# amolrpatil21/PorQua

Hardware: AMD Instinct MI355X
Metric: QPs solved/sec (rebalance dates) at N=1000 assets, 1-8 GPU; x vs host CPU (higher is better)
Workload: dtype f64; 1 GPU; config3: long-only min-variance (P=2*Pearson cov, budget + box [0,1]), daily rebalance; n_assets=1000, window=252, dates_per_gpu=4749, global_batch=4749, parallelism=dates-sharded x1

## Files before the change

### include/porqua_hip.h

```cpp
#ifndef PORQUA_HIP_H
#define PORQUA_HIP_H

#include <stdint.h>

#ifdef __cplusplus
extern "C" {
#endif

#define PQ_VERSION 100

#define PQ_UNSOLVED 0
#define PQ_SOLVED 1
#define PQ_SOLVED_INACCURATE 2
#define PQ_MAX_ITER 3
#define PQ_NEED_REFACTOR 4
#define PQ_PRIMAL_INFEASIBLE (-3)
#define PQ_DUAL_INFEASIBLE (-4)
#define PQ_NON_CONVEX (-5)

#define PQ_OUT_OBJ 0
#define PQ_OUT_PRIM 1
#define PQ_OUT_DUAL 2
#define PQ_OUT_GAP 3
#define PQ_OUT_RHO 4
// ... 137 lines not shown
int pq_admm_lr_grouped(const pq_lowrank* lr, const pq_problem* pb, pq_state* st, const double* Minv,
                       int32_t k_ld, int64_t M_stride, const int32_t* gdates, int32_t ngroups,
                       const int32_t* urows, const int32_t* ucnt, const int32_t* uoff, int32_t umax,
                       const pq_settings* s, int32_t iters_this_call, const double* pc, int64_t ldpc,
                       int32_t r0, const double* cc, const int32_t* cg_nzr, const double* cg_nzv,
                       int32_t nzmax, void* stream);

int pq_admm_lr_sweep(const pq_lowrank* lr, const pq_problem* pb, pq_state* st, const double* Minv,
                     int32_t k_ld, int64_t M_stride, const int32_t* gdates, int32_t ngroups,
                     const pq_settings* s, int32_t iters_this_call, const double* pc, int64_t ldpc,
                     int32_t r0, const double* cc, int32_t q_shared, double* scratch, int64_t scratch_doubles,
                     void* stream);
int64_t pq_sweep_scratch_doubles(int32_t n, int32_t batch, int32_t ngroups);

typedef struct pq_gcap {
  const int32_t* gdates; int32_t ngroups;
  const int32_t* urows; const int32_t* ucnt; const int32_t* uoff; int32_t umax;
  const int32_t* gidx;
  double* grho;
  double* M; double* Minv; int32_t k_ld; int64_t M_stride;
  double* aq; int64_t aq_stride;
  double* hinv; int32_t ldh;
  int32_t gmax;
} pq_gcap;
int pq_gcap_assemble(const pq_lowrank* lr, const pq_problem* pb, const pq_gcap* gc, const pq_settings* s,
                     const double* band, int64_t ldo, int32_t r0, const double* pc, int64_t ldpc,
                     const double* cc, void* stream);
int pq_gcap_prepare(const pq_lowrank* lr, const pq_problem* pb, pq_state* st, const pq_gcap* gc,
                    const pq_settings* s, const int32_t* idx, int32_t nidx, const double* band, int64_t ldo,
                    int32_t r0, const double* pc, int64_t ldpc, void* stream);
int pq_admm_lr_gcap(const pq_lowrank* lr, const pq_problem* pb, pq_state* st, const pq_gcap* gc,
                    const pq_settings* s, int32_t iters_this_call, const double* pc, int64_t ldpc, int32_t r0,
                    const double* cc, const int32_t* cg_nzr, const double* cg_nzv, int32_t nzmax, void* stream);

int pq_eigcap_form(const pq_lowrank* lr, const pq_problem* pb, const pq_state* st, const pq_settings* s,
                   const int32_t* pdate, const double* V, const double* evals, const double* What,
                   const double* cc, int32_t k_ld, const int32_t* idx, int32_t nidx, double* Minv,
                   int64_t M_stride, double* scratch, void* stream);

int pq_polish_batched(const pq_problem* pb, pq_state* st, const int32_t* idx, int32_t nidx,
                      const pq_settings* s, void* stream);

int pq_polish_lr_batched(const pq_lowrank* lr, const pq_problem* pb, pq_state* st,
                         const int32_t* idx, int32_t nidx, const pq_settings* s, void* stream);

int pq_polish_w_batched(const pq_lowrank* lr, const pq_problem* pb, pq_state* st, const int32_t* idx,
                        int32_t nidx, const pq_settings* s, int32_t ldk, int32_t final_try,
                        const double* band, int64_t ldo, int32_t r0, void* stream);

#define PQ_PG_RECORD 384
#define PQ_PG_PASS_SCRATCH 123537
#define PQ_PG_PENDING 0
#define PQ_PG_DONE 1
#define PQ_PG_FALLBACK 2
#define PQ_PG_SKIP 3
#define PQ_PG_WMB 8
#define PQ_PG_WSCR(k_ld) (2 * PQ_PG_WMB * (int64_t)(k_ld))
typedef struct pq_pg_wide {
  const pq_gcap* gc;
  const double* pc; int64_t ldpc; int32_t r0; const double* cc;
  const int32_t* nzr; const double* nzv; int32_t nzmax;
  double* wscr; int64_t wscr_stride;
  int32_t refine_steps;
} pq_pg_wide;
int pq_polish_grouped_init(const pq_lowrank* lr, const pq_problem* pb, pq_state* st, double* rec,
                           const pq_settings* s, void* stream);
// ... 97 lines not shown
```

### porqua_amd/_lib.py

```python
from __future__ import annotations

import ctypes
import os

_HERE = os.path.dirname(os.path.abspath(__file__))
LIB_PATH = os.environ.get("PQ_LIB_PATH") or os.path.join(_HERE, "libporqua_hip.so")

c_int32 = ctypes.c_int32
c_int64 = ctypes.c_int64
c_dp = ctypes.c_void_p

PQ_UNSOLVED = 0
PQ_SOLVED = 1
PQ_SOLVED_INACCURATE = 2
PQ_MAX_ITER = 3
PQ_NEED_REFACTOR = 4
PQ_PRIMAL_INFEASIBLE = -3
PQ_DUAL_INFEASIBLE = -4
PQ_NON_CONVEX = -5

PQ_PCT_OK, PQ_PCT_EMPTY_BUCKET, PQ_PCT_NAN_SCORE = range(3)
PQ_PCT_MAX_N = 16384
PQ_PCT_MAX_BUCKETS = 256

# ... 161 lines not shown
    "pq_admm_lr_grouped": ([ctypes.POINTER(PQLowRank), ctypes.POINTER(PQProblem), ctypes.POINTER(PQState),
                            c_dp, c_int32, c_int64, c_dp, c_int32, c_dp, c_dp, c_dp, c_int32,
                            ctypes.POINTER(PQSettings), c_int32, c_dp, c_int64, c_int32, c_dp, c_dp, c_dp,
                            c_int32, c_dp], c_int32),
    "pq_admm_lr_sweep": ([ctypes.POINTER(PQLowRank), ctypes.POINTER(PQProblem), ctypes.POINTER(PQState),
                          c_dp, c_int32, c_int64, c_dp, c_int32, ctypes.POINTER(PQSettings), c_int32, c_dp,
                          c_int64, c_int32, c_dp, c_int32, c_dp, c_int64, c_dp], c_int32),
    "pq_sweep_scratch_doubles": ([c_int32, c_int32, c_int32], c_int64),
    "pq_polish_lr_batched": ([ctypes.POINTER(PQLowRank), ctypes.POINTER(PQProblem), ctypes.POINTER(PQState),
                              c_dp, c_int32, ctypes.POINTER(PQSettings), c_dp], c_int32),
    "pq_lr_capacitance": ([ctypes.POINTER(PQLowRank), ctypes.POINTER(PQProblem), ctypes.POINTER(PQState),
                           c_dp, c_int32, ctypes.POINTER(PQSettings), c_dp, c_int32, c_int64, c_dp], c_int32),
    "pq_lr_band_gram": ([c_dp, c_int64, c_int32, c_int32, c_int32, c_int32, c_dp, c_int64, c_dp, c_int32, c_int32,
                         c_dp, c_int64, c_dp], c_int32),
    "pq_lr_capacitance_band": ([ctypes.POINTER(PQLowRank), ctypes.POINTER(PQProblem), ctypes.POINTER(PQState),
                                c_dp, c_int32, ctypes.POINTER(PQSettings), c_dp, c_int64, c_int32, c_dp, c_int64,
                                c_dp, c_dp, c_int32, c_int64, c_dp], c_int32),
    "pq_admm_lr_batched": ([ctypes.POINTER(PQLowRank), ctypes.POINTER(PQProblem), ctypes.POINTER(PQState),
                            c_dp, c_int32, c_int64, c_dp, c_int32, ctypes.POINTER(PQSettings), c_int32,
                            c_dp], c_int32),
    "pq_polish_grouped_init": ([ctypes.POINTER(PQLowRank), ctypes.POINTER(PQProblem), ctypes.POINTER(PQState),
                                c_dp, ctypes.POINTER(PQSettings), c_dp], c_int32),
    "pq_polish_grouped_round": ([ctypes.POINTER(PQLowRank), ctypes.POINTER(PQProblem), ctypes.POINTER(PQState),
                                 c_dp, c_int32, c_dp, c_int32, c_dp, c_dp, c_dp, c_int32,
                                 ctypes.POINTER(PQSettings), c_dp, ctypes.POINTER(PQPgWide), c_dp], c_int32),
    "pq_gcap_assemble": ([ctypes.POINTER(PQLowRank), ctypes.POINTER(PQProblem), ctypes.POINTER(PQGcap),
                          ctypes.POINTER(PQSettings), c_dp, c_int64, c_int32, c_dp, c_int64, c_dp, c_dp], c_int32),
    "pq_gcap_prepare": ([ctypes.POINTER(PQLowRank), ctypes.POINTER(PQProblem), ctypes.POINTER(PQState),
                         ctypes.POINTER(PQGcap), ctypes.POINTER(PQSettings), c_dp, c_int32, c_dp, c_int64, c_int32,
                         c_dp, c_int64, c_dp], c_int32),
    "pq_admm_lr_gcap": ([ctypes.POINTER(PQLowRank), ctypes.POINTER(PQProblem), ctypes.POINTER(PQState),
                         ctypes.POINTER(PQGcap), ctypes.POINTER(PQSettings), c_int32, c_dp, c_int64, c_int32, c_dp,
                         c_dp, c_dp, c_int32, c_dp], c_int32),
    "pq_eigcap_form": ([ctypes.POINTER(PQLowRank), ctypes.POINTER(PQProblem), ctypes.POINTER(PQState),
                        ctypes.POINTER(PQSettings), c_dp, c_dp, c_dp, c_dp, c_dp, c_int32, c_dp, c_int32, c_dp,
                        c_int64, c_dp, c_dp], c_int32),
    "pq_gemv_batched": ([c_dp, c_int64, c_int64, c_int32, c_int32, c_int32, c_int32, c_dp, c_int64, c_dp,
                         c_int64, c_dp], c_int32),
    "pq_workspace_bytes": ([c_int32, c_int32, c_int32, c_int32, c_int32, c_int32], c_int64),
    "pq_simulate_periods": ([c_dp, c_int64, c_int32, c_dp, c_int64, c_dp, c_dp, c_int32, c_dp, c_dp,
                             ctypes.c_double, ctypes.c_double, c_dp, c_dp, c_int64, c_dp, c_int32, c_dp], c_int32),
    "pq_lad_mv_batched": ([c_dp, c_int64, c_int64, c_int32, c_int32, c_dp, c_int64, c_int32, c_dp, c_int64,
                           c_dp, c_int64, c_dp], c_int32),
    "pq_wgram_batched": ([c_dp, c_int64, c_int64, c_int32, c_int32, c_int32, c_dp, c_int64, c_dp, c_int64,
                          c_dp, c_int64, c_dp, c_int32, c_int64, c_dp], c_int32),
    "pq_percentile_batched": ([c_dp, c_int64, c_int32, c_int32, ctypes.c_double, c_int32, c_dp, c_dp, c_dp,
                               c_dp, c_dp, c_dp, c_dp, c_dp, c_dp], c_int32),
    "pq_shrink_stats_band": ([c_dp, c_int64, c_int32, c_int32, c_int32, c_dp, c_int64, c_dp, c_int32, c_int32,
                              c_int32, c_int32, c_int32, c_dp, c_dp], c_int32),
    "pq_risk_parity_batched": ([ctypes.POINTER(PQLowRank), c_int32, c_int32, c_dp, c_dp, c_dp, c_int64,
                                ctypes.c_double, ctypes.c_double, c_int32, c_dp, c_int64, c_dp, c_dp, c_dp],
                               c_int32),
    "pq_hrp_batched": ([c_dp, c_int64, c_int32, c_int32, c_dp, c_dp, ctypes.c_double, c_dp, c_int64, c_dp, c_int64,
                        c_dp, c_dp, c_dp, c_dp], c_int32),
    "pq_hrp_linkage_batched": ([c_dp, c_int64, c_int32, c_int32, c_dp, c_dp, ctypes.c_double, c_int32, c_dp, c_int64,
                                c_dp, c_int64, c_dp, c_int64, c_dp, c_dp, c_dp, c_dp], c_int32),
    "pq_window_gram_batched": ([c_dp, c_int64, c_int32, c_dp, c_dp, c_int32, c_int32, c_dp, c_int64, c_dp, c_int32,
                                c_int64, c_dp], c_int32),
    "pq_window_project_batched": ([c_dp, c_int64, c_int32, c_dp, c_dp, c_int32, c_int32, c_dp, c_int64, c_dp,
                                   c_int32, c_int64, c_dp, c_dp, c_dp, c_int32, c_dp, c_dp, c_int64, c_dp], c_int32),
}

_lib = None


def load() -> ctypes.CDLL:
# ... 25 lines not shown
```

### porqua_amd/csrc/admm_gcap.hip

```cpp
#include "admm_dev.h"
#include "chol_dev.h"
#include "capi_util.h"

namespace pq {

constexpr int CT = 256;
constexpr int CNW = CT / 64;
constexpr int CHW = CT / 32;
constexpr int CTP1 = 5;
constexpr int CTP2 = 6;
constexpr int CG_MAX = 16;
constexpr int CU_MAX = 320;
constexpr int CMG = 4;
constexpr int CMGW = 24;
constexpr int CNZ = 4;
constexpr int CP1_ROWS = 16 * CNW * CTP1;
constexpr int CK_MAX = CP1_ROWS + 4;
constexpr int CH_MAX = 64;

#ifdef PQ_PROFILE
#define CSTAMP(k)                                                 \
  do {                                                            \
    __syncthreads();                                              \
    if (threadIdx.x == 0) {                                       \
// ... 364 lines not shown
      const int i = e >> 6, j = e & 63;
      T64[i * DP + j] = (i < mh && j < mh) ? h_entry(gg, i, j) : (i == j ? 1.0 : 0.0);
    }
    if (tile_chol_inv64(T64, X64, mh)) {
      if (t == 0) st.status[b] = PQ_NON_CONVEX;
      continue;
    }
    double* Hi = gc.hinv + (int64_t)b * gc.ldh * gc.ldh;
    const int ldh = gc.ldh;
    const int cc = l & 15, g4 = l >> 4;
    for (int tt = w; tt < 10; tt += PW_PREP) {
      int I = 0;
      while ((I + 1) * (I + 2) / 2 <= tt) ++I;
      const int J = tt - I * (I + 1) / 2;
      f64x4 acc = f64x4{0.0, 0.0, 0.0, 0.0};
#pragma unroll 4
      for (int k0 = 0; k0 < TB; k0 += 4)
        acc = __builtin_amdgcn_mfma_f64_16x16x4f64(X64[(16 * I + cc) * DP + k0 + g4], X64[(16 * J + cc) * DP + k0 + g4],
                                                  acc, 0, 0, 0);
#pragma unroll
      for (int q = 0; q < 4; ++q) {
        const int i = 16 * I + g4 + 4 * q, j = 16 * J + cc;
        const bool in = i < mh && j < mh;
        if (i < ldh && j < ldh) Hi[(int64_t)i * ldh + j] = in ? acc[q] : 0.0;
        if (I != J && i < ldh && j < ldh) Hi[(int64_t)j * ldh + i] = in ? acc[q] : 0.0;
      }
    }
  }
}

#ifndef PQ_GCAP_SKIP1
#define PQ_GCAP_SKIP1 1
#endif
template <int MGC, int NB>
__global__ __launch_bounds__(CT * NB) __attribute__((amdgpu_waves_per_eu(2, 2))) void k_admm_gcap(pq_lowrank lr, pq_problem pb, pq_state st, pq_gcap gc,
                                                  pq_settings s, int iters_call, const double* pc, int64_t ldpc,
                                                  int r0, const double* cc, const int32_t* cg_nzr,
                                                  const double* cg_nzv, int nzmax) {
  constexpr bool WIDE = MGC > CMG;
  constexpr int MGG = WIDE ? CMGW : 8;
  constexpr int CTN = CT * NB, CNWN = CTN / 64, CHWN = CTN / 32;
  constexpr int CG = CG_MAX * NB;
  constexpr int CTP1N = (CP1_ROWS / 16 + CNWN - 1) / CNWN;
  constexpr int CTP2N = ((CK_MAX + 15) / 16 + CNWN - 1) / CNWN;
  static_assert(CTP1N * CNWN * 16 >= CP1_ROWS && CTP2N * CNWN * 16 >= CK_MAX, "k_admm_gcap tiling");
  __shared__ __attribute__((aligned(16))) double WU[(CU_MAX + 4) * CG];
  double* const UT = WU;
  __shared__ double g_muv[CG], g_su[CG], g_dinv[CG], g_rn[CG], g_qmax[CG], g_coef[CG];
  __shared__ double g_y[CG * CH_MAX];
  constexpr int NPART = 5;
  __shared__ double g_part[CNWN * CG_MAX * NPART];
  __shared__ double g_gm[CG * 3];
  __shared__ double g_zg[CG * MGG], g_yg[CG * MGG], g_cgv[CG * MGG], g_cgx[CG * MGG],
      g_wg[CG * MGG], g_cw[CG * MGG], g_rgz[CG * MGG], g_cmu[CG * MGG];
  __shared__ double g_rg[MGG], g_lg[MGG], g_ug[MGG];
  double* const g_zt = g_rgz;
  __shared__ int g_act[CG], g_it[CG], g_end[CG], g_stat[CG], g_off[CG], g_T[CG];
  __shared__ int s_urow[CU_MAX];
  __shared__ double s_sr[MGG];
  __shared__ double s_rho;
  __shared__ int s_any;

  const int grp = xcd_slot(blockIdx.x, gridDim.x);
  const int d0 = gc.gdates[grp];
  const int G = gc.gdates[grp + 1] - d0;
  const int U = gc.ucnt[grp];
  const int t = threadIdx.x, w = wave_id(), l = lane_id();
  const int n = pb.n, ld = pb.ld, mg = pb.mg, k_ld = gc.k_ld;
  const int kU = U + mg;
  const bool has_box = pb.lb != nullptr;
  const bool centred = lr.mu != nullptr;
  const double sigma = s.sigma, alpha = s.alpha;
  const double* Mi = gc.Minv + (int64_t)grp * gc.M_stride;
#ifdef PQ_PROFILE
  long long pclk[5] = {0, 0, 0, 0, 0};
  long long tclk = wall_clock64();
#endif

  if (kU > CP1_ROWS || U > CU_MAX || G > CG || kU > k_ld) {
    for (int g = t; g < G; g += CTN) st.status[d0 + g] = PQ_NON_CONVEX;
    return;
  }

  for (int u = t; u < CU_MAX; u += CTN) s_urow[u] = u < U ? gc.urows[(int64_t)grp * gc.umax + u] : 0;
  for (int e = t; e < (CU_MAX + 4) * CG; e += CTN) UT[e] = 0.0;
  if (t == 0) s_rho = gc.grho[grp];
  __syncthreads();
  const double rho = s_rho;
  const GConst gk = gconst(lr, pb, s, d0, rho);
  if (t < mg) s_sr[t] = sqrt(row_rho(pb.lg[t], pb.ug[t], rho, s));
  if (t < CG) {
    const int g = t;
    int act = 0;
    if (g < G) {
      const int b = d0 + g;
      const int stt = st.status[b];
      act = (stt == PQ_UNSOLVED || stt == PQ_NEED_REFACTOR);
      g_it[g] = st.iters[b];
      g_end[g] = min(s.max_iter, st.iters[b] + iters_call);
      g_stat[g] = stt;
      g_T[g] = lr.tlen[b];
      g_off[g] = gc.uoff[b];
      g_dinv[g] = 1.0 / gk.d;
    }
    g_act[g] = act;
  }
  for (int e = t; e < CG * MGG; e += CTN) {
    const int g = e / MGG, r = e % MGG;
    double zg = 0, yg = 0;
    if (g < G && r < mg) {
      const int b = d0 + g;
      zg = st.z[(int64_t)b * st.m_ld + r];
      yg = st.y[(int64_t)b * st.m_ld + r];
    }
    g_zg[e] = zg;
    g_yg[e] = yg;
  }
  if (t < MGG) {
    const bool ok = t < mg;
    g_lg[t] = ok ? pb.lg[t] : 0.0;
    g_ug[t] = ok ? pb.ug[t] : 0.0;
    g_rg[t] = ok ? row_rho(pb.lg[t], pb.ug[t], rho, s) : 0.0;
// ... 63 lines not shown
      }
    }
    muv = lanes_sum<32>(muv);
    qmax = lanes_max<32>(qmax);
#pragma unroll
    for (int r = 0; r < CMG; ++r) cvp[r] = lanes_sum<32>(cvp[r]);
    if (hl == 0) {
      g_muv[g] = muv;
      g_qmax[g] = qmax;
      if constexpr (!WIDE)
        for (int r = 0; r < mg; ++r) g_cgv[g * MGG + r] = cvp[r];
    }
  }
  if (t == 0) {
    int any = 0;
    for (int g = 0; g < G; ++g) any |= g_act[g];
    s_any = any;
  }
  __syncthreads();

  const int ntile = (U + mg + 15) >> 4;
  const int ktile = (kU + 15) >> 4;
  while (s_any) {
#pragma clang diagnostic push
#pragma clang diagnostic ignored "-Wshadow"
    const int t = threadIdx.x + loop_zero();
    const int w = t >> 6, l = t & 63, hg = t >> 5, hl = t & 31;
    const int hbase = (hg & 1) * 32;
#pragma clang diagnostic pop
    (void)hbase;
    {
      const int z0 = loop_zero();
      const int kq = l >> 4, m0 = (l & 15) + z0;
      const double* Vp[NB];
      double wsc1[NB];
#pragma unroll
      for (int nb = 0; nb < NB; ++nb) {
        const int m = m0 + 16 * nb;
        Vp[nb] = (m < G) ? st.work + (int64_t)(d0 + m) * st.work_stride + ld : nullptr;
        wsc1[nb] = m < G ? g_dinv[m] : 1.0;
      }
      f64x4 c[CTP1N][NB];
      const double* arow[CTP1N];
      bool tv[CTP1N], aval[CTP1N];
      const int wu = __builtin_amdgcn_readfirstlane(w);
#pragma unroll
      for (int j = 0; j < CTP1N; ++j) {
#pragma unroll
        for (int nb = 0; nb < NB; ++nb) c[j][nb] = f64x4{0.0, 0.0, 0.0, 0.0};
        const int u = (w + CNWN * j) * 16 + m0;
        tv[j] = wu + CNWN * j < ntile;
        aval[j] = u < U + mg;
        arow[j] = u < U ? lr.panel + (int64_t)s_urow[u] * lr.ldp : pb.Cg + (int64_t)(u < U + mg ? u - U : 0) * ld;
      }
      struct Buf { double2 b[NB]; double2 a[CTP1N]; double bs[NB]; };
      const double* Vq[NB];
#pragma unroll
      for (int nb = 0; nb < NB; ++nb) Vq[nb] = Vp[nb] ? Vp[nb] : st.work + (int64_t)d0 * st.work_stride + ld;
      auto load = [&](Buf& f, int k0) {
        const int kk = k0 + 2 * kq;
        const bool kin = kk + 1 < n;
        const int kc = kin ? kk : 0;
#pragma unroll
        for (int nb = 0; nb < NB; ++nb) {
          f.b[nb] = *reinterpret_cast<const double2*>(Vq[nb] + kc);
          f.bs[nb] = (Vp[nb] && kin) ? 1.0 : 0.0;
        }
#pragma unroll
        for (int j = 0; j < CTP1N; ++j) f.a[j] = *reinterpret_cast<const double2*>(arow[j] + kc);
      };
      auto mma = [&](const Buf& f) {
#pragma unroll
        for (int nb = 0; nb < NB; ++nb) {
          const double bx = f.b[nb].x * f.bs[nb], by = f.b[nb].y * f.bs[nb];
#pragma unroll
          for (int j = 0; j < CTP1N; ++j) {
            if (PQ_GCAP_SKIP1 && !tv[j]) continue;
            c[j][nb] = __builtin_amdgcn_mfma_f64_16x16x4f64(f.a[j].x, bx, c[j][nb], 0, 0, 0);
            c[j][nb] = __builtin_amdgcn_mfma_f64_16x16x4f64(f.a[j].y, by, c[j][nb], 0, 0, 0);
          }
        }
      };
      Buf f0, f1;
      load(f0, 0);
      for (int k0 = 0; k0 < n; k0 += 16) {
        load(f1, k0 + 8);
        mma(f0);
        load(f0, k0 + 16);
        mma(f1);
      }
#pragma unroll
      for (int j = 0; j < CTP1N; ++j) {
        const int tile = w + CNWN * j;
        if (tv[j]) {
#pragma unroll
          for (int nb = 0; nb < NB; ++nb) {
            const int m = m0 + 16 * nb;
#pragma unroll
            for (int r = 0; r < 4; ++r) {
              const int u = tile * 16 + kq + 4 * r;
              if (u < U) {
                WU[u * CG + m] = gk.sqc * wsc1[nb] * c[j][nb][r];
              } else if (u < U + mg) {
                const double cgv = wsc1[nb] * c[j][nb][r];
                if (m < G) g_cgv[m * MGG + (u - U)] = cgv;
                WU[u * CG + m] = s_sr[u - U] * cgv;
              }
            }
          }
        }
      }
    }
    __syncthreads();
    CSTAMP(0);
    {
      const int z0 = loop_zero();
      const int kq = l >> 4, m = (l & 15) + z0;
      f64x4 z[CTP2N][NB];
      const double* mrow[CTP2N];
      bool zv[CTP2N], rv[CTP2N];
#pragma unroll
      for (int j = 0; j < CTP2N; ++j) {
#pragma unroll
        for (int nb = 0; nb < NB; ++nb) z[j][nb] = f64x4{0.0, 0.0, 0.0, 0.0};
        const int row = (w + CNWN * j) * 16 + m;
        zv[j] = w + CNWN * j < ktile;
        rv[j] = row < kU;
        mrow[j] = Mi + (int64_t)(rv[j] ? row : 0) * k_ld;
      }
      const int kU4 = (kU + 7) & ~7;
      auto loadA = [&](double2 (&a)[CTP2N], int k0) {
        const int kk = k0 + 2 * kq;
        const int k0c = kk < kU ? kk : 0, k1c = kk + 1 < kU ? kk + 1 : 0;
#pragma unroll
        for (int j = 0; j < CTP2N; ++j) {
          const int ts = zv[j] ? (w + CNWN * j) * 16 : 0;
          const bool left = kk < ts;
          const double* mc = Mi + (ts + m);
          a[j].x = *(left ? mrow[j] + kk : mc + (int64_t)k0c * k_ld);
          a[j].y = *(left ? mrow[j] + kk + 1 : mc + (int64_t)k1c * k_ld);
// ... 185 lines not shown
          double cwv = 0.0;
          for (int r2 = 0; r2 < mg; ++r2) cwv = fma(cc[r * mg + r2], g_cw[g * MGG + r2], cwv);
          if (hl == 0) g_zt[g * MGG + r] = g_cgv[g * MGG + r] - dinv * (a - su * g_cmu[g * MGG + r] + cwv);
        }
        __builtin_amdgcn_wave_barrier();
        double gm[3] = {0.0, 0.0, 0.0};
        if (hl < mg) {
          const int e = g * MGG + hl;
          const double rg = g_rg[hl], zt = g_zt[e];
          const RowStep rs = row_step(zt, g_zg[e], g_yg[e], rg, g_lg[hl], g_ug[hl], alpha);
          const double zn = rs.zn, yn = rs.yn;
          const double cx = alpha * zt + (1.0 - alpha) * g_cgx[e];
          gm[0] = fabs(cx - zn);
          gm[1] = fabs(cx);
          gm[2] = fabs(zn);
          g_rgz[e] = rg * zt;
          g_zg[e] = zn;
          g_yg[e] = yn;
          g_cgx[e] = cx;
          g_wg[e] = rg * zn - yn;
        }
#pragma unroll
        for (int k = 0; k < 3; ++k) gm[k] = lanes_max<32>(gm[k]);
        if (hl == 0)
          for (int k = 0; k < 3; ++k) g_gm[g * 3 + k] = gm[k];
      }
    }
    __syncthreads();
    CSTAMP(2);
    {
      const int z0 = loop_zero();
      const int kq = l >> 4, ia = (l & 15) + z0;
      const int Uk = (U + 3) & ~3;
      const int cb = w / CNW, wb = w - cb * CNW;
#ifndef PQ_GCAP_PS
#define PQ_GCAP_PS 4
#endif
      constexpr int PS = PQ_GCAP_PS;
      constexpr int NR = 4;
      bool mact[NR];
#pragma unroll
      for (int r = 0; r < NR; ++r) {
        const int m = 16 * cb + kq + 4 * r;
        mact[r] = m < G && g_act[m];
      }
      const bool box_shared = pb.box_stride == 0;
      double mv[NR][4];
      double muv[NR];
#pragma unroll
      for (int r = 0; r < NR; ++r) {
        muv[r] = 0.0;
#pragma unroll
        for (int e = 0; e < 4; ++e) mv[r][e] = 0.0;
      }
      for (int p = wb; p * 32 < n; p += CNW) {
        const int i = p * 32 + 2 * ia;
        const bool cin = i < n;
        f64x4 ce = f64x4{0.0, 0.0, 0.0, 0.0}, co = f64x4{0.0, 0.0, 0.0, 0.0};
        struct ABuf { double2 a[PS]; };
        auto load = [&](ABuf& f, int u0) {
#pragma unroll
          for (int h = 0; h < PS; ++h) {
            const int u = u0 + 4 * h + kq;
            f.a[h] = *reinterpret_cast<const double2*>(lr.panel + (int64_t)s_urow[u < U ? u : 0] * lr.ldp +
                                                       (cin ? i : 0));
          }
        };
        auto mma = [&](const ABuf& f, int u0) {
#pragma unroll
          for (int h = 0; h < PS; ++h) {
            const int u = u0 + 4 * h + kq;
            const double av = u < U ? UT[u * CG + 16 * cb + ia] : 0.0;
            ce = __builtin_amdgcn_mfma_f64_16x16x4f64(av, f.a[h].x, ce, 0, 0, 0);
            co = __builtin_amdgcn_mfma_f64_16x16x4f64(av, f.a[h].y, co, 0, 0, 0);
          }
        };
        ABuf f0, f1;
        load(f0, 0);
        for (int u0 = 0; u0 < Uk; u0 += 8 * PS) {
          load(f1, u0 + 4 * PS);
          mma(f0, u0);
          load(f0, u0 + 8 * PS);
          mma(f1, u0 + 4 * PS);
        }
        if (!cin) continue;
        constexpr int MGL = WIDE ? 0 : MGC;
        constexpr int MGR = MGL > 0 ? MGL : 1;
        double2 cg2[MGR];
#pragma unroll
        for (int c = 0; c < MGL; ++c)
          cg2[c] = c < mg ? *reinterpret_cast<const double2*>(pb.Cg + (int64_t)c * ld + i) : double2{0.0, 0.0};
        int nzr2[2][WIDE ? CNZ : 1];
        double nzv2[2][WIDE ? CNZ : 1];
        if constexpr (WIDE) {
#pragma unroll
          for (int h = 0; h < 2; ++h)
#pragma unroll
            for (int e = 0; e < CNZ; ++e) {
              const bool ok = e < nzmax;
              nzr2[h][e] = ok ? cg_nzr[(int64_t)(i + h) * nzmax + e] : -1;
              nzv2[h][e] = ok ? cg_nzv[(int64_t)(i + h) * nzmax + e] : 0.0;
            }
        }
        double2 lo2 = double2{0.0, 0.0}, up2 = double2{0.0, 0.0}, rb2 = double2{0.0, 0.0};
        if (has_box && box_shared) {
          lo2 = *reinterpret_cast<const double2*>(pb.lb + i);
          up2 = *reinterpret_cast<const double2*>(pb.ub + i);
          rb2 = double2{row_rho(lo2.x, up2.x, rho, s), row_rho(lo2.y, up2.y, rho, s)};
        }
#pragma unroll
        for (int r = 0; r < NR; ++r) {
          __builtin_amdgcn_sched_barrier(0);
          if (!mact[r]) continue;
          const int m = 16 * cb + kq + 4 * r;
          const int bm = d0 + m;
          const double su = g_su[m], dinv = g_dinv[m];
          double2 lo = lo2, up = up2, rb = rb2;
          if (has_box && !box_shared) {
            lo = *reinterpret_cast<const double2*>(pb.lb + (int64_t)bm * pb.box_stride + i);
            up = *reinterpret_cast<const double2*>(pb.ub + (int64_t)bm * pb.box_stride + i);
            rb = double2{row_rho(lo.x, up.x, rho, s), row_rho(lo.y, up.y, rho, s)};
          }
          double* R_m = st.work + (int64_t)bm * st.work_stride + ld + i;
          double* x_m = st.x + (int64_t)bm * ld + i;
          double* Px_m = st.Px + (int64_t)bm * ld + i;
          double* zb_m = st.z + (int64_t)bm * st.m_ld + st.mg_pad + i;
          double* yb_m = st.y + (int64_t)bm * st.m_ld + st.mg_pad + i;
          const double2 rr2 = *reinterpret_cast<const double2*>(R_m);
          const double2 mu2 = centred ? *reinterpret_cast<const double2*>(lr.mu + (int64_t)bm * lr.mu_stride + i)
                                      : double2{0.0, 0.0};
          const double2 x2 = *reinterpret_cast<const double2*>(x_m);
          const double2 px2 = *reinterpret_cast<const double2*>(Px_m);
          const double2 q2 = *reinterpret_cast<const double2*>(pb.q + (int64_t)bm * pb.q_stride + i);
          double2 z2 = double2{0.0, 0.0}, y2 = double2{0.0, 0.0};
          if (has_box) {
            z2 = *reinterpret_cast<const double2*>(zb_m);
            y2 = *reinterpret_cast<const double2*>(yb_m);
          }
          double cwm[MGR], rgzm[MGR], ygm[MGR], wgm[MGR];
#pragma unroll
          for (int c = 0; c < MGL; ++c) {
            const bool ok = c < mg;
            cwm[c] = ok ? g_cw[m * MGG + c] : 0.0;
            rgzm[c] = ok ? g_rgz[m * MGG + c] : 0.0;
            ygm[c] = ok ? g_yg[m * MGG + c] : 0.0;
            wgm[c] = ok ? g_wg[m * MGG + c] : 0.0;
          }
// ... 25 lines not shown
            }
            const double xt = (rr0 - corr) * dinv;
            double pxt = rr0 - sigma * xt - rbi * xt - grgz;
#pragma unroll
            for (int c = 0; c < MGL; ++c) {
              pxt -= cgi[c] * rgzm[c];
              cgy = fma(cgi[c], ygm[c], cgy);
              cgw = fma(cgi[c], wgm[c], cgw);
            }
            const double xn = alpha * xt + (1.0 - alpha) * xi;
            const double pxn = alpha * pxt + (1.0 - alpha) * pxi;
            double rr = sigma * xn - qi + cgw;
            double cty = 0.0;
            zn_o = zi;
            yn_o = yi;
            if (has_box) {
              const RowStep rs = row_step(xt, zi, yi, rbi, loi, upi, alpha);
              const double zn = rs.zn, yn = rs.yn;
              zn_o = zn;
              yn_o = yn;
              cty = yn;
              rr += rbi * zn - yn;
              mv[r][0] = fmax(mv[r][0], fabs(xn - zn));
              mv[r][1] = fmax(mv[r][1], fmax(fabs(xn), fabs(zn)));
            }
            xn_o = xn;
            pxn_o = pxn;
            rr_o = rr;
            const double cy = cty + cgy;
            mv[r][2] = fmax(mv[r][2], fabs((pxn + qi + cty) + (cy - cty)));
            mv[r][3] = fmax(mv[r][3], fmax(fabs(pxn), fabs(cy)));
            muv[r] = fma(mui, rr * dinv, muv[r]);
          };
          one(ce[r], rr2.x, mu2.x, x2.x, px2.x, q2.x, z2.x, y2.x, lo.x, up.x, rb.x, 0, xo.x, pxo.x, zo.x, yo.x, ro.x);
          one(co[r], rr2.y, mu2.y, x2.y, px2.y, q2.y, z2.y, y2.y, lo.y, up.y, rb.y, 1, xo.y, pxo.y, zo.y, yo.y, ro.y);
          *reinterpret_cast<double2*>(x_m) = xo;
          *reinterpret_cast<double2*>(Px_m) = pxo;
          *reinterpret_cast<double2*>(R_m) = ro;
          if (has_box) {
            *reinterpret_cast<double2*>(zb_m) = zo;
            *reinterpret_cast<double2*>(yb_m) = yo;
          }
        }
      }
#pragma unroll
      for (int r = 0; r < NR; ++r) {
#pragma unroll
        for (int sh = 1; sh < 16; sh <<= 1) {
#pragma unroll
          for (int e = 0; e < 4; ++e) mv[r][e] = fmax(mv[r][e], __shfl_xor(mv[r][e], sh, 64));
          muv[r] += __shfl_xor(muv[r], sh, 64);
        }
        const int m = 16 * cb + kq + 4 * r;
        if (ia == 0) {
          double* pp = g_part + (w * CG_MAX + (m - 16 * cb)) * NPART;
#pragma unroll
          for (int e = 0; e < 4; ++e) pp[e] = mv[r][e];
          pp[4] = muv[r];
        }
      }
    }
    __syncthreads();
    CSTAMP(3);
    if (t < G && g_act[t]) {
      const int g = t;
      double mv[7] = {g_gm[g * 3], fmax(g_gm[g * 3 + 1], g_gm[g * 3 + 2]), 0.0, 0.0, 0.0, 0.0, g_qmax[g]};
      double muv = 0.0;
      for (int ww = (g / 16) * CNW; ww < (g / 16 + 1) * CNW; ++ww) {
        const double* pp = g_part + (ww * CG_MAX + (g & 15)) * NPART;
        mv[0] = fmax(mv[0], pp[0]);
        mv[1] = fmax(mv[1], pp[1]);
        mv[3] = fmax(mv[3], pp[2]);
        mv[4] = fmax(mv[4], pp[3]);
        muv += pp[4];
      }
      const int it = g_it[g] + 1;
      int stat = PQ_UNSOLVED;
      const bool finite = isfinite(muv);
      const double eps_p = eps_prim(mv, s), eps_d = eps_dual(mv, s);
      double rn = 0.0;
      if (!finite) {
        stat = PQ_NON_CONVEX;
      } else if (it >= s.min_iter && mv[0] <= eps_p && mv[3] <= eps_d) {
        stat = PQ_SOLVED;
      } else if (s.adapt_interval > 0 && it % s.adapt_interval == 0) {
        rn = rho_request(mv, rho, s);
      }
      if (stat == PQ_UNSOLVED && it >= s.max_iter) stat = PQ_MAX_ITER;
      g_it[g] = it;
      g_stat[g] = stat;
      g_act[g] = (stat == PQ_UNSOLVED) && it < g_end[g];
      g_rn[g] = rn;
      g_muv[g] = muv;
    }
    __syncthreads();
    if (t == 0) {
      double lsum = 0.0;
      int nreq = 0;
      for (int g = 0; g < G; ++g)
        if (g_rn[g] > 0.0 && g_stat[g] == PQ_UNSOLVED) { lsum += log(g_rn[g]); ++nreq; }
      int adapt = 0;
      if (nreq) {
// ... 34 lines not shown
      const int b = d0 + g;
      st.z[(int64_t)b * st.m_ld + r] = g_zg[e];
      st.y[(int64_t)b * st.m_ld + r] = g_yg[e];
    }
  }
#ifdef PQ_PROFILE
  if (t == 0) {
    for (int g = 0; g < G; ++g) {
      double* dstp = st.work + (int64_t)(d0 + g) * st.work_stride + PQ_WORK_PROF(ld, st.mg_pad) + 16;
      for (int k2 = 0; k2 < 5; ++k2) dstp[k2] += (double)pclk[k2] / G;
    }
  }
#endif
#undef GC_HPTRS
}

}

static int gcap_check(const pq_lowrank* lr, const pq_problem* pb, const pq_gcap* gc, const char* who) {
  PQ_CHECK_ARG(lr && pb && gc, "%s: null argument", who);
  PQ_CHECK_ARG(gc->gdates && gc->urows && gc->ucnt && gc->uoff && gc->gidx && gc->grho && gc->ngroups > 0,
               "%s: group plan missing", who);
  PQ_CHECK_ARG(gc->umax > 0 && gc->umax <= pq::CU_MAX, "%s: umax must be in (0, %d]", who, pq::CU_MAX);
  PQ_CHECK_ARG(pb->mg >= 0 && pb->mg <= pq::CMGW && pb->Cg_stride == 0 && pb->g_stride == 0,
               "%s: needs shared general rows, mg <= %d", who, pq::CMGW);
  PQ_CHECK_ARG(gc->k_ld % 64 == 0 && gc->k_ld >= 64 && gc->k_ld <= 384,
               "%s: need 64 <= k_ld <= 384, a multiple of 64 (k_ld=%d)", who, gc->k_ld);
  PQ_CHECK_ARG(gc->gmax >= 0 && gc->gmax <= pq::CG_MAX * 2, "%s: gmax must be in [0, %d] (gmax=%d)", who,
               pq::CG_MAX * 2, gc->gmax);
  return 0;
}

static int gcap_nb(const pq_gcap* gc) { return gc->gmax > pq::CG_MAX ? 2 : 1; }

extern "C" int pq_gcap_assemble(const pq_lowrank* lr, const pq_problem* pb, const pq_gcap* gc,
                                const pq_settings* s, const double* band, int64_t ldo, int32_t r0,
                                const double* pc, int64_t ldpc, const double* cc, void* stream) {
  if (gcap_check(lr, pb, gc, "pq_gcap_assemble")) return -1;
  PQ_CHECK_ARG(s && band && gc->M, "pq_gcap_assemble: null argument");
  PQ_CHECK_ARG(pb->mg == 0 || (pc && cc), "pq_gcap_assemble: general rows need pc and cc");
  static const int old_form = [] {
    const char* e = getenv("PQ_GCAP_ASSEMBLE_OLD");
    return e ? atoi(e) : 0;
  }();
  const int nb = gc->k_ld / 64;
  if (old_form > 0)
    hipLaunchKernelGGL(pq::k_gcap_assemble_rows, dim3(gc->ngroups), dim3(256), 0, (hipStream_t)stream, *lr, *pb, *gc,
                       *s, band, ldo, r0, pc, ldpc, cc);
  else
    hipLaunchKernelGGL(pq::k_gcap_assemble, dim3(gc->ngroups * (nb * (nb + 1) / 2)), dim3(256), 0, (hipStream_t)stream,
                       *lr, *pb, *gc, *s, band, ldo, r0, pc, ldpc, cc);
  PQ_CHECK_LAUNCH("pq_gcap_assemble");
  return 0;
}

extern "C" int pq_gcap_prepare(const pq_lowrank* lr, const pq_problem* pb, pq_state* st, const pq_gcap* gc,
                               const pq_settings* s, const int32_t* idx, int32_t nidx, const double* band,
                               int64_t ldo, int32_t r0, const double* pc, int64_t ldpc, void* stream) {
  if (gcap_check(lr, pb, gc, "pq_gcap_prepare")) return -1;
  PQ_CHECK_ARG(st && s && band && gc->Minv && gc->aq && gc->hinv, "pq_gcap_prepare: null argument");
  PQ_CHECK_ARG(gc->aq_stride >= 2 * (int64_t)gc->k_ld && gc->ldh > 0 && gc->ldh <= pq::CH_MAX,
               "pq_gcap_prepare: aq needs 2 k_ld per date, ldh <= %d", pq::CH_MAX);
  PQ_CHECK_ARG(pb->mg == 0 || pc, "pq_gcap_prepare: general rows need pc");
  PQ_CHECK_ARG(gc->umax <= pq::CU_MAX && pb->mg <= pq::CMGW, "pq_gcap_prepare: union or general rows too many");
  const int grid = idx ? nidx : gc->ngroups;
  if (grid <= 0) return 0;
  static const int skip = [] {
    const char* e = getenv("PQ_PREP_SKIP");
    return e ? atoi(e) : 0;
  }();
  if (gcap_nb(gc) == 2)
    hipLaunchKernelGGL(pq::k_gcap_prep<2>, dim3(grid), dim3(pq::PT_PREP), 0, (hipStream_t)stream, *lr, *pb, *st, *gc,
                       *s, idx, band, ldo, r0, pc, ldpc, skip);
  else
    hipLaunchKernelGGL(pq::k_gcap_prep<1>, dim3(grid), dim3(pq::PT_PREP), 0, (hipStream_t)stream, *lr, *pb, *st, *gc,
                       *s, idx, band, ldo, r0, pc, ldpc, skip);
  PQ_CHECK_LAUNCH("pq_gcap_prepare");
  return 0;
}

extern "C" int pq_admm_lr_gcap(const pq_lowrank* lr, const pq_problem* pb, pq_state* st, const pq_gcap* gc,
                               const pq_settings* s, int32_t iters_this_call, const double* pc, int64_t ldpc,
                               int32_t r0, const double* cc, const int32_t* cg_nzr, const double* cg_nzv,
                               int32_t nzmax, void* stream) {
  if (gcap_check(lr, pb, gc, "pq_admm_lr_gcap")) return -1;
  PQ_CHECK_ARG(st && s && gc->Minv && gc->aq && gc->hinv, "pq_admm_lr_gcap: null argument");
  PQ_CHECK_ARG(pb->mg == 0 || (pc && cc), "pq_admm_lr_gcap: general rows need pc and cc");
  PQ_CHECK_ARG(pb->n % 2 == 0 && lr->ldp % 2 == 0, "pq_admm_lr_gcap: needs even n and panel stride");
  PQ_CHECK_ARG(st->work && st->work_stride >= 3 * (int64_t)pb->ld, "pq_admm_lr_gcap: work buffer too small");
  PQ_CHECK_ARG(pb->ld % 2 == 0 && st->work_stride % 2 == 0 && st->m_ld % 2 == 0 && st->mg_pad % 2 == 0 &&
                   pb->q_stride % 2 == 0 && pb->box_stride % 2 == 0 && lr->mu_stride % 2 == 0,
               "pq_admm_lr_gcap: strides must be even");
  PQ_CHECK_ARG(pb->mg <= pq::CMG || (cg_nzr && cg_nzv && nzmax > 0 && nzmax <= pq::CNZ),
               "pq_admm_lr_gcap: more than %d general rows need their column-sparse form (nzmax <= %d)", pq::CMG,
               pq::CNZ);
  const dim3 grid(gc->ngroups);
  const hipStream_t str = (hipStream_t)stream;
  if (gcap_nb(gc) == 2) {
    const dim3 blk(pq::CT * 2);
    if (pb->mg == 0)
      hipLaunchKernelGGL((pq::k_admm_gcap<0, 2>), grid, blk, 0, str, *lr, *pb, *st, *gc, *s, iters_this_call, pc, ldpc,
                         r0, cc, nullptr, nullptr, 0);
    else if (pb->mg == 1)
      hipLaunchKernelGGL((pq::k_admm_gcap<1, 2>), grid, blk, 0, str, *lr, *pb, *st, *gc, *s, iters_this_call, pc, ldpc,
                         r0, cc, nullptr, nullptr, 0);
    else if (pb->mg <= pq::CMG)
      hipLaunchKernelGGL((pq::k_admm_gcap<pq::CMG, 2>), grid, blk, 0, str, *lr, *pb, *st, *gc, *s, iters_this_call, pc,
                         ldpc, r0, cc, nullptr, nullptr, 0);
    else
      hipLaunchKernelGGL((pq::k_admm_gcap<pq::CMGW, 2>), grid, blk, 0, str, *lr, *pb, *st, *gc, *s, iters_this_call, pc,
                         ldpc, r0, cc, cg_nzr, cg_nzv, nzmax);
  } else {
    const dim3 blk(pq::CT);
    if (pb->mg == 0)
      hipLaunchKernelGGL((pq::k_admm_gcap<0, 1>), grid, blk, 0, str, *lr, *pb, *st, *gc, *s, iters_this_call, pc, ldpc,
                         r0, cc, nullptr, nullptr, 0);
    else if (pb->mg == 1)
      hipLaunchKernelGGL((pq::k_admm_gcap<1, 1>), grid, blk, 0, str, *lr, *pb, *st, *gc, *s, iters_this_call, pc, ldpc,
                         r0, cc, nullptr, nullptr, 0);
    else if (pb->mg <= pq::CMG)
      hipLaunchKernelGGL((pq::k_admm_gcap<pq::CMG, 1>), grid, blk, 0, str, *lr, *pb, *st, *gc, *s, iters_this_call, pc,
                         ldpc, r0, cc, nullptr, nullptr, 0);
    else
      hipLaunchKernelGGL((pq::k_admm_gcap<pq::CMGW, 1>), grid, blk, 0, str, *lr, *pb, *st, *gc, *s, iters_this_call, pc,
                         ldpc, r0, cc, cg_nzr, cg_nzv, nzmax);
  }
  PQ_CHECK_LAUNCH("pq_admm_lr_gcap");
  return 0;
}
```

Measured before the change: 765,700 QPs/s.

## Add tail form for groups of up to 20 dates in gcap ADMM kernel

Adds a third kernel form for date groups slightly larger than 16 (up to 16+4). The four extra tail dates are handled with scalar FMA accumulations and cross-lane shuffles instead of a second full 16-wide MFMA column block. In the update phase all waves cover the whole panel range, with a fifth row slot for the tail dates. The goal is to cut MFMA work and panel traffic that a full 32-date form spends on mostly empty columns. The cost is extra VALU FMAs, shuffles, LDS reads and more code complexity. The form is on by default and can be turned off with an environment variable.

```diff
diff --git a/include/porqua_hip.h b/include/porqua_hip.h
--- a/include/porqua_hip.h
+++ b/include/porqua_hip.h
@@ -193,6 +193,7 @@
 int pq_admm_lr_gcap(const pq_lowrank* lr, const pq_problem* pb, pq_state* st, const pq_gcap* gc,
                     const pq_settings* s, int32_t iters_this_call, const double* pc, int64_t ldpc, int32_t r0,
                     const double* cc, const int32_t* cg_nzr, const double* cg_nzv, int32_t nzmax, void* stream);
+int pq_gcap_form(int32_t gmax, int32_t mg);
 
 int pq_eigcap_form(const pq_lowrank* lr, const pq_problem* pb, const pq_state* st, const pq_settings* s,
                    const int32_t* pdate, const double* V, const double* evals, const double* What,
diff --git a/porqua_amd/_lib.py b/porqua_amd/_lib.py
--- a/porqua_amd/_lib.py
+++ b/porqua_amd/_lib.py
@@ -217,6 +217,7 @@
     "pq_admm_lr_gcap": ([ctypes.POINTER(PQLowRank), ctypes.POINTER(PQProblem), ctypes.POINTER(PQState),
                          ctypes.POINTER(PQGcap), ctypes.POINTER(PQSettings), c_int32, c_dp, c_int64, c_int32, c_dp,
                          c_dp, c_dp, c_int32, c_dp], c_int32),
+    "pq_gcap_form": ([c_int32, c_int32], c_int32),
     "pq_eigcap_form": ([ctypes.POINTER(PQLowRank), ctypes.POINTER(PQProblem), ctypes.POINTER(PQState),
                         ctypes.POINTER(PQSettings), c_dp, c_dp, c_dp, c_dp, c_dp, c_int32, c_dp, c_int32, c_dp,
                         c_int64, c_dp, c_dp], c_int32),
diff --git a/porqua_amd/csrc/admm_gcap.hip b/porqua_amd/csrc/admm_gcap.hip
--- a/porqua_amd/csrc/admm_gcap.hip
+++ b/porqua_amd/csrc/admm_gcap.hip
@@ -420,13 +420,24 @@
 #ifndef PQ_GCAP_SKIP1
 #define PQ_GCAP_SKIP1 1
 #endif
-template <int MGC, int NB>
+constexpr int CRT = 4;
+#ifndef PQ_GCAP_TAIL_P1
+#define PQ_GCAP_TAIL_P1 0
+#endif
+template <int MGC, int NB, int TL = 0>
 __global__ __launch_bounds__(CT * NB) __attribute__((amdgpu_waves_per_eu(2, 2))) void k_admm_gcap(pq_lowrank lr, pq_problem pb, pq_state st, pq_gcap gc,
                                                   pq_settings s, int iters_call, const double* pc, int64_t ldpc,
                                                   int r0, const double* cc, const int32_t* cg_nzr,
                                                   const double* cg_nzv, int nzmax) {
   constexpr bool WIDE = MGC > CMG;
   constexpr int MGG = WIDE ? CMGW : 8;
+  constexpr bool TAIL = TL > 0;
+  static_assert(!TAIL || NB == 2, "the tail form is a 32-date form");
+  constexpr bool TAIL1 = TAIL && PQ_GCAP_TAIL_P1 != 0;
+  constexpr int NB1 = TAIL1 ? 1 : NB;
+  constexpr int RT1 = TAIL1 ? CRT : 1;
+  constexpr int RT = TAIL ? CRT : 1;
+  constexpr int GP = TAIL ? CG_MAX + CRT : CG_MAX;
   constexpr int CTN = CT * NB, CNWN = CTN / 64, CHWN = CTN / 32;
   constexpr int CG = CG_MAX * NB;
   constexpr int CTP1N = (CP1_ROWS / 16 + CNWN - 1) / CNWN;
@@ -437,7 +448,7 @@
   __shared__ double g_muv[CG], g_su[CG], g_dinv[CG], g_rn[CG], g_qmax[CG], g_coef[CG];
   __shared__ double g_y[CG * CH_MAX];
   constexpr int NPART = 5;
-  __shared__ double g_part[CNWN * CG_MAX * NPART];
+  __shared__ double g_part[CNWN * GP * NPART];
   __shared__ double g_gm[CG * 3];
   __shared__ double g_zg[CG * MGG], g_yg[CG * MGG], g_cgv[CG * MGG], g_cgx[CG * MGG],
       g_wg[CG * MGG], g_cw[CG * MGG], g_rgz[CG * MGG], g_cmu[CG * MGG];
@@ -465,7 +476,7 @@
   long long tclk = wall_clock64();
 #endif
 
-  if (kU > CP1_ROWS || U > CU_MAX || G > CG || kU > k_ld) {
+  if (kU > CP1_ROWS || U > CU_MAX || G > (TAIL ? CG_MAX + CRT : CG) || kU > k_ld) {
     for (int g = t; g < G; g += CTN) st.status[d0 + g] = PQ_NON_CONVEX;
     return;
   }
@@ -475,7 +486,13 @@
   if (t == 0) s_rho = gc.grho[grp];
   __syncthreads();
   const double rho = s_rho;
-  const GConst gk = gconst(lr, pb, s, d0, rho);
+  GConst gk = gconst(lr, pb, s, d0, rho);
+  if constexpr (TAIL) {
+    gk.c = readlane_f64(gk.c, 0);
+    gk.sqc = readlane_f64(gk.sqc, 0);
+    gk.d = readlane_f64(gk.d, 0);
+    gk.rho = readlane_f64(gk.rho, 0);
+  }
   if (t < mg) s_sr[t] = sqrt(row_rho(pb.lg[t], pb.ug[t], rho, s));
   if (t < CG) {
     const int g = t;
@@ -605,52 +622,76 @@
     {
       const int z0 = loop_zero();
       const int kq = l >> 4, m0 = (l & 15) + z0;
-      const double* Vp[NB];
-      double wsc1[NB];
-#pragma unroll
-      for (int nb = 0; nb < NB; ++nb) {
+      const double* Vp[NB1];
+      double wsc1[NB1];
+#pragma unroll
+      for (int nb = 0; nb < NB1; ++nb) {
         const int m = m0 + 16 * nb;
         Vp[nb] = (m < G) ? st.work + (int64_t)(d0 + m) * st.work_stride + ld : nullptr;
         wsc1[nb] = m < G ? g_dinv[m] : 1.0;
       }
-      f64x4 c[CTP1N][NB];
+      f64x4 c[CTP1N][NB1];
+      double ta[CTP1N][RT1];
       const double* arow[CTP1N];
       bool tv[CTP1N], aval[CTP1N];
       const int wu = __builtin_amdgcn_readfirstlane(w);
 #pragma unroll
       for (int j = 0; j < CTP1N; ++j) {
 #pragma unroll
-        for (int nb = 0; nb < NB; ++nb) c[j][nb] = f64x4{0.0, 0.0, 0.0, 0.0};
+        for (int nb = 0; nb < NB1; ++nb) c[j][nb] = f64x4{0.0, 0.0, 0.0, 0.0};
+#pragma unroll
+        for (int d = 0; d < RT1; ++d) ta[j][d] = 0.0;
         const int u = (w + CNWN * j) * 16 + m0;
         tv[j] = wu + CNWN * j < ntile;
         aval[j] = u < U + mg;
         arow[j] = u < U ? lr.panel + (int64_t)s_urow[u] * lr.ldp : pb.Cg + (int64_t)(u < U + mg ? u - U : 0) * ld;
       }
-      struct Buf { double2 b[NB]; double2 a[CTP1N]; double bs[NB]; };
-      const double* Vq[NB];
-#pragma unroll
-      for (int nb = 0; nb < NB; ++nb) Vq[nb] = Vp[nb] ? Vp[nb] : st.work + (int64_t)d0 * st.work_stride + ld;
+      struct Buf { double2 b[NB1]; double2 a[CTP1N]; double bs[NB1]; double2 t[RT1]; double ks; };
+      const double* Vq[NB1];
+#pragma unroll
+      for (int nb = 0; nb < NB1; ++nb) Vq[nb] = Vp[nb] ? Vp[nb] : st.work + (int64_t)d0 * st.work_stride + ld;
+      const double* Vt[RT1];
+#pragma unroll
+      for (int d = 0; d < RT1; ++d)
+        Vt[d] = st.work + (int64_t)(d0 + z0 + (TAIL1 && CG_MAX + d < G ? CG_MAX + d : 0)) * st.work_stride + ld;
       auto load = [&](Buf& f, int k0) {
         const int kk = k0 + 2 * kq;
         const bool kin = kk + 1 < n;
         const int kc = kin ? kk : 0;
 #pragma unroll
-        for (int nb = 0; nb < NB; ++nb) {
+        for (int nb = 0; nb < NB1; ++nb) {
           f.b[nb] = *reinterpret_cast<const double2*>(Vq[nb] + kc);
           f.bs[nb] = (Vp[nb] && kin) ? 1.0 : 0.0;
+        }
+        if constexpr (TAIL1) {
+#pragma unroll
+          for (int d = 0; d < RT1; ++d) f.t[d] = *reinterpret_cast<const double2*>(Vt[d] + kc);
+          f.ks = kin ? 1.0 : 0.0;
         }
 #pragma unroll
         for (int j = 0; j < CTP1N; ++j) f.a[j] = *reinterpret_cast<const double2*>(arow[j] + kc);
       };
       auto mma = [&](const Buf& f) {
 #pragma unroll
-        for (int nb = 0; nb < NB; ++nb) {
+        for (int nb = 0; nb < NB1; ++nb) {
           const double bx = f.b[nb].x * f.bs[nb], by = f.b[nb].y * f.bs[nb];
 #pragma unroll
           for (int j = 0; j < CTP1N; ++j) {
             if (PQ_GCAP_SKIP1 && !tv[j]) continue;
             c[j][nb] = __builtin_amdgcn_mfma_f64_16x16x4f64(f.a[j].x, bx, c[j][nb], 0, 0, 0);
             c[j][nb] = __builtin_amdgcn_mfma_f64_16x16x4f64(f.a[j].y, by, c[j][nb], 0, 0, 0);
+          }
+        }
+        if constexpr (TAIL1) {
+#pragma unroll
+          for (int d = 0; d < RT1; ++d) {
+            const double tx = f.t[d].x * f.ks, ty = f.t[d].y * f.ks;
+#pragma unroll
+            for (int j = 0; j < CTP1N; ++j) {
+              if (PQ_GCAP_SKIP1 && !tv[j]) continue;
+              ta[j][d] = fma(f.a[j].x, tx, ta[j][d]);
+              ta[j][d] = fma(f.a[j].y, ty, ta[j][d]);
+            }
           }
         }
       };
@@ -667,7 +708,7 @@
         const int tile = w + CNWN * j;
         if (tv[j]) {
 #pragma unroll
-          for (int nb = 0; nb < NB; ++nb) {
+          for (int nb = 0; nb < NB1; ++nb) {
             const int m = m0 + 16 * nb;
 #pragma unroll
             for (int r = 0; r < 4; ++r) {
@@ -679,6 +720,26 @@
                 if (m < G) g_cgv[m * MGG + (u - U)] = cgv;
                 WU[u * CG + m] = s_sr[u - U] * cgv;
               }
+            }
+          }
+          if constexpr (TAIL1) {
+            double tsel = 0.0;
+#pragma unroll
+            for (int d = 0; d < RT1; ++d) {
+              double x = ta[j][d];
+              x += __shfl_xor(x, 16, 64);
+              x += __shfl_xor(x, 32, 64);
+              tsel = kq == d ? x : tsel;
+            }
+            const int m = CG_MAX + kq, u = tile * 16 + m0;
+            const bool live = m < G;
+            const double wsc = live ? g_dinv[live ? m : 0] : 0.0;
+            if (u < U) {
+              WU[u * CG + m] = live ? gk.sqc * wsc * tsel : 0.0;
+            } else if (u < U + mg) {
+              const double cgv = wsc * tsel;
+              if (live) g_cgv[m * MGG + (u - U)] = cgv;
+              WU[u * CG + m] = live ? s_sr[u - U] * cgv : 0.0;
             }
           }
         }
@@ -930,12 +991,13 @@
       const int z0 = loop_zero();
       const int kq = l >> 4, ia = (l & 15) + z0;
       const int Uk = (U + 3) & ~3;
-      const int cb = w / CNW, wb = w - cb * CNW;
+      const int cb = TAIL ? 0 : w / CNW, wb = w - cb * CNW;
+      constexpr int PSTEP = TAIL ? CNWN : CNW;
 #ifndef PQ_GCAP_PS
 #define PQ_GCAP_PS 4
 #endif
       constexpr int PS = PQ_GCAP_PS;
-      constexpr int NR = 4;
+      constexpr int NR = TAIL ? 5 : 4;
       bool mact[NR];
 #pragma unroll
       for (int r = 0; r < NR; ++r) {
@@ -951,10 +1013,13 @@
 #pragma unroll
         for (int e = 0; e < 4; ++e) mv[r][e] = 0.0;
       }
-      for (int p = wb; p * 32 < n; p += CNW) {
+      for (int p = wb; p * 32 < n; p += PSTEP) {
         const int i = p * 32 + 2 * ia;
         const bool cin = i < n;
         f64x4 ce = f64x4{0.0, 0.0, 0.0, 0.0}, co = f64x4{0.0, 0.0, 0.0, 0.0};
+        double2 te[RT];
+#pragma unroll
+        for (int d = 0; d < RT; ++d) te[d] = double2{0.0, 0.0};
         struct ABuf { double2 a[PS]; };
         auto load = [&](ABuf& f, int u0) {
 #pragma unroll
@@ -971,6 +1036,18 @@
             const double av = u < U ? UT[u * CG + 16 * cb + ia] : 0.0;
             ce = __builtin_amdgcn_mfma_f64_16x16x4f64(av, f.a[h].x, ce, 0, 0, 0);
             co = __builtin_amdgcn_mfma_f64_16x16x4f64(av, f.a[h].y, co, 0, 0, 0);
+            if constexpr (TAIL) {
+              static_assert(CRT == 4, "two 16-byte LDS reads per union row");
+              const double2* tp = reinterpret_cast<const double2*>(UT + (u < U ? u : 0) * CG + CG_MAX);
+              const double2 t01 = tp[0], t23 = tp[1];
+              const double us = u < U ? 1.0 : 0.0;
+              const double tv4[4] = {t01.x * us, t01.y * us, t23.x * us, t23.y * us};
+#pragma unroll
+              for (int d = 0; d < RT; ++d) {
+                te[d].x = fma(tv4[d], f.a[h].x, te[d].x);
+                te[d].y = fma(tv4[d], f.a[h].y, te[d].y);
+              }
+            }
           }
         };
         ABuf f0, f1;
@@ -981,7 +1058,20 @@
           load(f0, u0 + 8 * PS);
           mma(f1, u0 + 4 * PS);
         }
+        double2 tsel = double2{0.0, 0.0};
+        if constexpr (TAIL) {
+#pragma unroll
+          for (int d = 0; d < RT; ++d) {
+            double x = te[d].x, y = te[d].y;
+            x += __shfl_xor(x, 16, 64);
+            y += __shfl_xor(y, 16, 64);
+            x += __shfl_xor(x, 32, 64);
+            y += __shfl_xor(y, 32, 64);
+            tsel = kq == d ? double2{x, y} : tsel;
+          }
+        }
         if (!cin) continue;
+        const int kqe = TAIL ? kq + loop_zero() : kq;
         constexpr int MGL = WIDE ? 0 : MGC;
         constexpr int MGR = MGL > 0 ? MGL : 1;
         double2 cg2[MGR];
@@ -1010,7 +1100,7 @@
         for (int r = 0; r < NR; ++r) {
           __builtin_amdgcn_sched_barrier(0);
           if (!mact[r]) continue;
-          const int m = 16 * cb + kq + 4 * r;
+          const int m = 16 * cb + kqe + 4 * r;
           const int bm = d0 + m;
           const double su = g_su[m], dinv = g_dinv[m];
           double2 lo = lo2, up = up2, rb = rb2;
@@ -1102,8 +1192,9 @@
             mv[r][3] = fmax(mv[r][3], fmax(fabs(pxn), fabs(cy)));
             muv[r] = fma(mui, rr * dinv, muv[r]);
           };
-          one(ce[r], rr2.x, mu2.x, x2.x, px2.x, q2.x, z2.x, y2.x, lo.x, up.x, rb.x, 0, xo.x, pxo.x, zo.x, yo.x, ro.x);
-          one(co[r], rr2.y, mu2.y, x2.y, px2.y, q2.y, z2.y, y2.y, lo.y, up.y, rb.y, 1, xo.y, pxo.y, zo.y, yo.y, ro.y);
+          const double xre = r < 4 ? ce[r < 4 ? r : 0] : tsel.x, xro = r < 4 ? co[r < 4 ? r : 0] : tsel.y;
+          one(xre, rr2.x, mu2.x, x2.x, px2.x, q2.x, z2.x, y2.x, lo.x, up.x, rb.x, 0, xo.x, pxo.x, zo.x, yo.x, ro.x);
+          one(xro, rr2.y, mu2.y, x2.y, px2.y, q2.y, z2.y, y2.y, lo.y, up.y, rb.y, 1, xo.y, pxo.y, zo.y, yo.y, ro.y);
           *reinterpret_cast<double2*>(x_m) = xo;
           *reinterpret_cast<double2*>(Px_m) = pxo;
           *reinterpret_cast<double2*>(R_m) = ro;
@@ -1123,7 +1214,7 @@
         }
         const int m = 16 * cb + kq + 4 * r;
         if (ia == 0) {
-          double* pp = g_part + (w * CG_MAX + (m - 16 * cb)) * NPART;
+          double* pp = g_part + (w * GP + (m - 16 * cb)) * NPART;
 #pragma unroll
           for (int e = 0; e < 4; ++e) pp[e] = mv[r][e];
           pp[4] = muv[r];
@@ -1136,8 +1227,9 @@
       const int g = t;
       double mv[7] = {g_gm[g * 3], fmax(g_gm[g * 3 + 1], g_gm[g * 3 + 2]), 0.0, 0.0, 0.0, 0.0, g_qmax[g]};
       double muv = 0.0;
-      for (int ww = (g / 16) * CNW; ww < (g / 16 + 1) * CNW; ++ww) {
-        const double* pp = g_part + (ww * CG_MAX + (g & 15)) * NPART;
+      const int ww0 = TAIL ? 0 : (g / 16) * CNW, ww1 = TAIL ? CNWN : (g / 16 + 1) * CNW;
+      for (int ww = ww0; ww < ww1; ++ww) {
+        const double* pp = g_part + (ww * GP + (TAIL ? g : (g & 15))) * NPART;
         mv[0] = fmax(mv[0], pp[0]);
         mv[1] = fmax(mv[1], pp[1]);
         mv[3] = fmax(mv[3], pp[2]);
@@ -1238,6 +1330,13 @@
 }
 
 static int gcap_nb(const pq_gcap* gc) { return gc->gmax > pq::CG_MAX ? 2 : 1; }
+
+extern "C" int pq_gcap_form(int32_t gmax, int32_t mg) {
+  if (gmax <= pq::CG_MAX) return 1;
+  if (gmax > pq::CG_MAX + pq::CRT || mg > pq::CMG) return 2;
+  const char* e = getenv("PQ_GCAP_TAIL");
+  return (e && atoi(e) == 0) ? 2 : 3;
+}
 
 extern "C" int pq_gcap_assemble(const pq_lowrank* lr, const pq_problem* pb, const pq_gcap* gc,
                                 const pq_settings* s, const double* band, int64_t ldo, int32_t r0,
@@ -1302,7 +1401,19 @@
                pq::CNZ);
   const dim3 grid(gc->ngroups);
   const hipStream_t str = (hipStream_t)stream;
-  if (gcap_nb(gc) == 2) {
+  const int form = pq_gcap_form(gc->gmax, pb->mg);
+  if (form == 3) {
+    const dim3 blk(pq::CT * 2);
+    if (pb->mg == 0)
+      hipLaunchKernelGGL((pq::k_admm_gcap<0, 2, 1>), grid, blk, 0, str, *lr, *pb, *st, *gc, *s, iters_this_call, pc,
+                         ldpc, r0, cc, nullptr, nullptr, 0);
+    else if (pb->mg == 1)
+      hipLaunchKernelGGL((pq::k_admm_gcap<1, 2, 1>), grid, blk, 0, str, *lr, *pb, *st, *gc, *s, iters_this_call, pc,
+                         ldpc, r0, cc, nullptr, nullptr, 0);
+    else
+      hipLaunchKernelGGL((pq::k_admm_gcap<pq::CMG, 2, 1>), grid, blk, 0, str, *lr, *pb, *st, *gc, *s, iters_this_call,
+                         pc, ldpc, r0, cc, nullptr, nullptr, 0);
+  } else if (form == 2) {
     const dim3 blk(pq::CT * 2);
     if (pb->mg == 0)
       hipLaunchKernelGGL((pq::k_admm_gcap<0, 2>), grid, blk, 0, str, *lr, *pb, *st, *gc, *s, iters_this_call, pc, ldpc,
```

Result: faster. 791,200 QPs/s (median of 6 runs) (+3.3%).
